# adjerbetian/OpenCL_PathTracer

Hardware: AMD Instinct MI355X
Metric: Msamples/s (paths x bounces) at 1920x1080 (higher is better)
Workload: dtype f32; 1 GPU; BASELINE configs[2]: synthetic random-triangle scene (numpy MT19937 seed 12345): 1000000 triangles (665533 BVH nodes, depth 22), 1920x1080, ray depth 10, JITTERED, 1 light(s); spp_total=256, parallelism=single GPU

## Files before the change

opencl_pathtracer_amd/csrc/kernel_wavefront.hip:

```cpp
#include <hip/hip_runtime.h>

#include "leaf_cull.h"
#include "ptmi_device.hpp"
#include "ptmi_shading.hpp"
#include "ptmi_literal_path.hpp"

#include <atomic>
#include <cstdlib>
#include <cstring>

namespace PTMI_DEV_NS {

constexpr int kWfBlock = 256;
constexpr int kWfBlockNarrow = 64;
constexpr int kWfStack = PTMI_BVH_MAX_DEPTH;
#ifndef PTMI_WF_MIN_WAVES
#define PTMI_WF_MIN_WAVES 5
#endif
#ifndef PTMI_WF_MIN_WAVES_GENERAL
#define PTMI_WF_MIN_WAVES_GENERAL 5
#endif
#ifndef PTMI_WF_QUEUES
#define PTMI_WF_QUEUES 8
#endif
// ... 258 lines not shown
            asm volatile("" ::: "memory");
            Ray wr;
            wr.o = v4(fetch(r.o.x), fetch(r.o.y), fetch(r.o.z), fetch(r.o.w));
            wr.d = v4(fetch(r.d.x), fetch(r.d.y), fetch(r.d.z), fetch(r.d.w));
            wr.ix = wr.iy = wr.iz = 0;
            const float w_limit = fetch(limit);
            if (has_item) {
                unsigned long long* const owner_key = &key_mem[wave_first + owner];
                tri_test<PRE>(e0, e1, [&](float4& l0, float4& l1) { l0 = rec[kL0]; l1 = rec[kL1]; }, wr, w_limit,
                              [&](const V4&, float ray_t, float s, float t, bool front, float nsd) {
                    const bool nan_hit = NANSAFE && !w_shadow && !(nsd == nsd);
                    const unsigned long long key = w_shadow ? ((unsigned long long)w_tri << 32)
                                                   : nan_hit ? 0ull
                                                   : (((unsigned long long)__float_as_uint(nsd) << 32) | (unsigned long long)(~w_tri));
                    atomicMin(owner_key, key);
                    if (!w_shadow && *owner_key == key) {
                        uint32_t* const rec_out = &stack_mem[wave_first + owner];
                        rec_out[0 * kWfBlock] = __float_as_uint(ray_t);
                        rec_out[kWordS * kWfBlock] = __float_as_uint(s);
                        rec_out[kWordT * kWfBlock] = __float_as_uint(t);
                        rec_out[kWordTri * kWfBlock] = w_tri | (front ? kHitFront : 0u) | kHitFound;
                    }
                });
            }
        }
        if (cnt != 0u) {
            const uint32_t won = (uint32_t)(key_mem[tid] >> 32);
            if (NANSAFE && !shadow && won == 0u) {
                give_path_up(radiance, transfer, reflection, p_bbx, p_tri);
                hit_mem[kWordTri * kWfBlock] = 0;
                cur = REF_NONE; tri_i = tri_end = 0; sp = stack_floor;
                if (kTos) tos = REF_NONE;
                job_counter[1] = 1u;
            } else
            if (!shadow) {
                limit = __uint_as_float(won);
                p_tri += cnt; tri_i += cnt;
            } else if (won != 0xFFFFFFFFu) {
                p_tri += won - tri_i + 1u;
                hit_mem[kWordTri * kWfBlock] |= kHitFound;
                tri_end = tri_i; cur = REF_NONE;
            } else {
                p_tri += cnt; tri_i += cnt;
            }
            if (tri_i >= tri_end && ref_is_leaf(cur)) enter_leaf(false);
        }
    };
    auto node_step = [&]() {
        const float4* const rec = reinterpret_cast<const float4*>(&sc.tris[cur & REF_INDEX_MASK_INNER]);
        const float4 a = rec[0], b = rec[1], c = rec[2], d = rec[3];
        const NodeView n = node_view(a, b, c, d);
        const bool fwd = ((dir_signs >> n.axis) & 1u) != 0;
        float d2_1 = 0, d2_2 = 0;
        if (kCull) {
            d2_1 = ptmi_cull::box_distance2(n.lo1, n.hi1, r.o.x, r.o.y, r.o.z);
            d2_2 = ptmi_cull::box_distance2(n.lo2, n.hi2, r.o.x, r.o.y, r.o.z);
            asm volatile("" : "+v"(d2_1), "+v"(d2_2));
        }
        bool h1, h2;
        if (!wave_exact) {
            h1 = box_hit_ordered(n.lo1, n.hi1, r, limit);
            h2 = box_hit_ordered(n.lo2, n.hi2, r, limit);
        } else {
            h1 = box_hit(n.lo1, n.hi1, (n.ref1 & REF_EMPTY) != 0, r, limit);
            h2 = box_hit(n.lo2, n.hi2, (n.ref2 & REF_EMPTY) != 0, r, limit);
        }
        p_bbx += 2;
        bool culled = false;
        if (kCull) {
            const uint32_t cull_bits = n.cull & (dir_signs >> 3) & sc.leaf_cull;
            const bool first = fwd ? h1 : !h2;
            const bool certified = (cull_bits & (first ? ptmi_cull::kCullChild1 : ptmi_cull::kCullChild2)) != 0u;
            culled = (h1 | h2) & certified & ptmi_cull::box_is_beyond(first ? d2_1 : d2_2, limit);
        }
        const uint32_t far_ref = fwd ? n.ref2 : n.ref1;
        sp[kWfBlock] = far_ref;
        uint32_t* const pushed = sp + kWfBlock;
        const uint32_t child = fwd ? (h1 ? n.ref1 : n.ref2) : (h2 ? n.ref2 : n.ref1);
        cur = h1 ? child : (h2 ? child : cur);
        if (kTos) tos = h1 ? (h2 ? far_ref : tos) : tos;
        sp = h1 ? (h2 ? pushed : sp) : sp;
        if (!(h1 | h2)) pop();
        if (ref_is_leaf(cur)) enter_leaf(culled);
    };

    int wait_debt = 0;
    bool pending, want_inner, want_post;
    int n_t, n_i, n_p;
    bool any_lane;
    unsigned long long dead_lanes = 0ull;
    auto survey = [&]() {
        pending = tri_i < tri_end;
        const bool has_node = cur < REF_DEAD;
        const unsigned long long b_t = __builtin_amdgcn_ballot_w64(pending), b_n = __builtin_amdgcn_ballot_w64(has_node), b_dead = dead_lanes;
        const unsigned long long m_t = b_t, m_i = b_n & ~b_t, m_p = ~(b_t | b_n | b_dead);
        want_inner = !pending & has_node;
        want_post = !pending & !has_node & (cur != REF_DEAD);
        any_lane = (m_t | m_i | m_p) != 0ull;
        n_t = __popcll(m_t); n_i = __popcll(m_i); n_p = __popcll(m_p);
        asm volatile("" : "+s"(n_t), "+s"(n_i));
        wait_debt += n_p;
    };
    const int wait_debt_bound = (int)sc.wait_debt;
    auto path_logic_due = [&]() { return n_p > 0 && wait_debt >= wait_debt_bound; };
    auto nothing_traverses = [&]() { return n_t == 0 && n_i == 0; };
    for (;;) {
        survey();
        if (!any_lane) break;
        auto to_path_logic = [&]() { return path_logic_due() || nothing_traverses(); };
        auto pass_is_due = [&]() { return n_t >= kLeafLanes || (n_t > 0 && 3 * n_t >= kLeafRatio * n_i); };
        while (!to_path_logic()) {
            if (pass_is_due()) {
                leaf_pass(pending);
                survey();
                continue;
            }
            if (STATS) { trips_i++; lanes_i += n_i; }
            if (want_inner) node_step();
            survey();
        }
        wait_debt = 0;
        if (STATS) { trips_p++; lanes_p += n_p; }
        const unsigned long long pass_start = STATS ? __builtin_amdgcn_s_memtime() : 0ull;
        bool new_ray = false;
        V4 new_direction = v4(0, 0, 0, 0);
        if (want_post) {
            need_path = cur == REF_IDLE;
            alive = true;
            bool end_path = false, missed = false;
            bool start_shadow = false, do_scatter = false, lit = false;
            Hit hit;
            hit.point = v4(0, 0, 0, 0); hit.s = hit.t = 0; hit.tri = 0; hit.front = false;
            if (!need_path) {
// ... 101 lines not shown
                    got_job = gx < sc.width && gy < sc.height;
                }
            }
            if (open && base + n_want > q_size) {
                q_cur = (q_cur + 1u) % (uint32_t)kQueues;
                q_done++;
            }
        }

        if (want_post) {
            if (got_job) {
                const uint32_t it = first_iteration + it_local * iteration_stride;
                slot = it_local * (sc.width * sc.height) + gy * sc.width + gx;
                seed = lcg_seed(gx, gy, sc.width, sc.height, it, sc.source_seed != 0);
                float sample_x, sample_y;
                draw_sample(sc, gx, gy, it, seed, sample_x, sample_y);
                check(sample_x >= -0.5f && sample_y >= -0.5f && sample_x <= 0.5f && sample_y <= 0.5f, C_CHK_SAMPLE);
                {
                    const DScene& cs = cold_scene();
                    r.o = v4(cs.cam_pos);
                    new_direction = mad(v4(cs.cam_up), sample_y, mad(v4(cs.cam_right), sample_x, v4(cs.cam_dir)));
                }
                radiance = v4(0, 0, 0, 0);
                transfer = v4(1, 1, 1, 1);
                reflection = 0; p_bbx = 0; p_tri = 0;
                in_water = false;
                shadow = false;
                need_path = false;
                bool skip = false;
                if (SS && it > 5u) {
                    const DScene& cs = cold_scene();
                    const uint32_t off = owns_pixel ? gy * sc.width + gx : sample_pixel(sc, sample_x, sample_y);
                    const float n = cs.image_ray_nb[off];
                    const float4 vv = reinterpret_cast<const float4*>(cs.image_v)[off];
                    const float sigma2_n = fmaxf(fmaxf(fdiv(vv.x, n), fdiv(vv.y, n)), fdiv(vv.z, n));
                    uint32_t idx = (uint32_t)n;
                    if (idx > 1000u) idx = 1000u;
                    skip = (double)lcg_random(seed) > (double)fdiv(100 * sigma2_n, cs.x2inv[idx]) + 0.05;
                }
                if (skip) {
                    if (owns_pixel) cold_scene().stage_flag[gy * sc.width + gx] = 0.f;
                    need_path = true;
                } else
                if (sc.max_depth > 0) {
                    limit = INFINITY;
                    new_ray = true;
                } else {
                    finish_path(false);
                }
            }
            if (new_ray) {
                ray_set_direction(r, new_direction);
                dir_signs = (r.d.x > 0 ? 1u : 0u) | (r.d.y > 0 ? 2u : 0u) | (r.d.z > 0 ? 4u : 0u);
                if (kCull && ptmi_cull::ray_may_cull(r.o.x, r.o.y, r.o.z, r.o.w, r.d.w)) dir_signs |= (ptmi_cull::kCullChild1 | ptmi_cull::kCullChild2) << 3;
                const float o_size = __builtin_fabsf(r.o.x) + __builtin_fabsf(r.o.y) + __builtin_fabsf(r.o.z) + __builtin_fabsf(r.o.w);
                const float d_size = __builtin_fabsf(r.d.x) + __builtin_fabsf(r.d.y) + __builtin_fabsf(r.d.z) + __builtin_fabsf(r.d.w);
                bool bad = !((o_size <= 0x1p+40f) & (d_size <= 4.0f));
                if (!PLAIN && !owns_pixel && __builtin_expect(bad, 0)) {
                    const uint32_t place = atomicAdd(&job_counter[2], 1u);
                    bad = place < kGiveUpListCap;
                    if (bad) {
                        job_counter[kGiveUpListFirst + place] = slot;
                        slot |= kGivenUp;
                    }
                }
                if (__builtin_expect(bad, 0)) {
                    give_path_up(radiance, transfer, reflection, p_bbx, p_tri);
                    shadow = false;
                    job_counter[1] = 1u;
                }
                start_query();
                if (__builtin_expect(bad, 0)) { cur = REF_NONE; tri_i = tri_end = 0; }
            }
            if (need_path) cur = alive ? REF_IDLE : REF_DEAD;
        }
        dead_lanes = __builtin_amdgcn_ballot_w64(cur == REF_DEAD);
        wave_exact = __builtin_amdgcn_ballot_w64(exact_boxes) != 0ull;
        if (STATS) cycles_p += __builtin_amdgcn_s_memtime() - pass_start;
    }

    if (STATS && (tid & 63u) == 0) {
        atomicAdd(&block_counters[C_TRIPS_I], (unsigned long long)trips_i);
        atomicAdd(&block_counters[C_LANES_I], lanes_i);
        atomicAdd(&block_counters[C_TRIPS_T], (unsigned long long)(pass_rounds));
        atomicAdd(&block_counters[C_LANES_T], (unsigned long long)pass_items);
        atomicAdd(&block_counters[C_TRIPS_P], (unsigned long long)trips_p);
        atomicAdd(&block_counters[C_LANES_P], lanes_p);
        atomicAdd(&block_counters[C_CYCLES_P], cycles_p);
        atomicAdd(&block_counters[C_CYCLES_LOOP], __builtin_amdgcn_s_memtime() - loop_start);
    }
    if (STATS && culled_items != 0u) atomicAdd(&block_counters[C_LANES_T], (unsigned long long)culled_items);
    if (STATS && item_violations != 0u) atomicAdd(&block_counters[C_ITEM_VIOLATIONS], (unsigned long long)item_violations);
    __syncthreads();
    if (tid < (STATS ? 1u : (uint32_t)PTMI_COUNTER_SPLITS)) {
        unsigned long long* const totals = &block_counters[tid * kSplitWords];
        totals[C_SHADOW] = totals[C_HITS] * sc.n_lights;
    }
    __syncthreads();
    if (STATS) {
        if (tid < C_COUNT) atomicAdd(&cold_scene().counters[tid], block_counters[tid]);
    } else if (tid < kBlockCounters) {
        const uint32_t k = tid / kSplitWords, c = tid % kSplitWords;
        if (k == 0u || block_counters[tid] != 0ull) atomicAdd(&cold_scene().counters[k * C_COUNT + c], block_counters[tid]);
    }
}

template <bool PRE>
// ... 380 lines not shown
```

opencl_pathtracer_amd/csrc/leaf_cull.h:

```cpp
#ifndef PTMI_LEAF_CULL_H
#define PTMI_LEAF_CULL_H

#include <cmath>
#include <cstdint>

#include "ptmi_internal.h"

namespace ptmi_cull {

constexpr float kRel = 1.001f, kAbs = 0.01f, kMaxOrigin = 0x1p+41f;
constexpr double kKappaMax = 0x1p-13, kEpsAbsMax = 2.0e-3;

constexpr uint32_t kCullChild1 = 1u, kCullChild2 = 2u, kCullComputed = 4u;

PTMI_HD float box_distance2(const float lo[3], const float hi[3], float ox, float oy, float oz)
{
    const float dx = fmaxf(fmaxf(lo[0] - ox, ox - hi[0]), 0.0f);
    const float dy = fmaxf(fmaxf(lo[1] - oy, oy - hi[1]), 0.0f);
    const float dz = fmaxf(fmaxf(lo[2] - oz, oz - hi[2]), 0.0f);
    return fmaf(dz, dz, fmaf(dy, dy, dx * dx));
}

PTMI_HD bool ray_may_cull(float ox, float oy, float oz, float ow, float dw)
{
    return fabsf(ox) + fabsf(oy) + fabsf(oz) <= kMaxOrigin && ow == 1.0f && dw == 0.0f;
}
PTMI_HD bool box_is_beyond(float d2, float limit)
{
    return d2 > fmaf(limit, kRel, kAbs);
}
PTMI_HD bool leaf_cull_rule(float d2, float limit, float ox, float oy, float oz, float ow, float dw)
{
    return box_is_beyond(d2, limit) && ray_may_cull(ox, oy, oz, ow, dw);
}

PTMI_HD bool triangle_slack(const ptmi_triangle& t, const float lo[3], const float hi[3], double* eps_abs, double* kappa)
{
    const double u24 = 0x1p-24;
    const float S[3][3] = {{t.s1.x, t.s1.y, t.s1.z}, {t.s2.x, t.s2.y, t.s2.z}, {t.s3.x, t.s3.y, t.s3.z}};
    if (!(t.s1.w == t.s2.w && t.s1.w == t.s3.w && fabsf(t.s1.w) <= 0x1p+20f)) return false;
    if (!(t.n.w == 0.0f || (t.s1.w == 1.0f && fabsf(t.n.w) <= 4.0f))) return false;
    double B2 = 0;
    for (int k = 0; k < 3; k++) {
        if (!(lo[k] <= hi[k] && fabsf(lo[k]) <= 0x1p+20f && fabsf(hi[k]) <= 0x1p+20f)) return false;
        for (int j = 0; j < 3; j++)
            if (!(S[j][k] >= lo[k] && S[j][k] <= hi[k])) return false;
        const double m = fmax(fabs((double)lo[k]), fabs((double)hi[k]));
        B2 += m * m;
    }
    const double B = sqrt(B2);
    const float uf[3] = {S[1][0] - S[0][0], S[1][1] - S[0][1], S[1][2] - S[0][2]}, vf[3] = {S[2][0] - S[0][0], S[2][1] - S[0][1], S[2][2] - S[0][2]};
    const float uv_c = fmaf(uf[2], vf[2], fmaf(uf[1], vf[1], uf[0] * vf[0])), uu_c = fmaf(uf[2], uf[2], fmaf(uf[1], uf[1], uf[0] * uf[0])),
                vv_c = fmaf(vf[2], vf[2], fmaf(vf[1], vf[1], vf[0] * vf[0]));
    const double ud[3] = {uf[0], uf[1], uf[2]}, vd[3] = {vf[0], vf[1], vf[2]};
    const double uu = ud[0] * ud[0] + ud[1] * ud[1] + ud[2] * ud[2], vv = vd[0] * vd[0] + vd[1] * vd[1] + vd[2] * vd[2],
                 uv = ud[0] * vd[0] + ud[1] * vd[1] + ud[2] * vd[2];
    const double lu = sqrt(uu), lv = sqrt(vv);
    if (!(lu >= 0x1p-16 && lv >= 0x1p-16)) return false;
    const double cr[3] = {ud[1] * vd[2] - ud[2] * vd[1], ud[2] * vd[0] - ud[0] * vd[2], ud[0] * vd[1] - ud[1] * vd[0]};
    const double area2 = sqrt(cr[0] * cr[0] + cr[1] * cr[1] + cr[2] * cr[2]);
    if (!(area2 > 0)) return false;
    const double N[3] = {t.n.x, t.n.y, t.n.z};
    const double Nn = (N[0] * cr[0] + N[1] * cr[1] + N[2] * cr[2]) / area2, len_n = sqrt(N[0] * N[0] + N[1] * N[1] + N[2] * N[2]);
    if (!(fabs(Nn) >= 0.25 && len_n <= 4.0)) return false;
    const double tan2 = len_n * len_n - Nn * Nn;
    const double tilt = sqrt(tan2 > 0 ? tan2 : 0) / fabs(Nn);
    if (!(tilt <= 0x1p-18)) return false;
    const float det_c[2] = {uv_c * uv_c - uu_c * vv_c, fmaf(uv_c, uv_c, -(uu_c * vv_c))};
    double dk = 0, c_w = 0;
    for (int m = 0; m < 2; m++) {
        if (!(det_c[m] < 0.0f)) return false;
        const double den = (double)(1.0f / det_c[m]);
        if (!std::isfinite(den)) return false;
// ... 47 lines not shown
```

opencl_pathtracer_amd/csrc/ptmi_api.cpp:

```cpp
#include <cstdlib>
#include <cstring>
#include <mutex>

#include "ptmi_context.h"

using namespace ptmi_internal;

namespace {
std::mutex g_err_mutex;
std::string g_err;
}

void ptmi_internal::set_global_error(const std::string& msg)
{
    std::lock_guard<std::mutex> lock(g_err_mutex);
    g_err = msg;
}

extern "C" {

int ptmi_abi_version(void) { return PTMI_ABI_VERSION; }

int ptmi_device_count(void)
{
// ... 19 lines not shown
        return fail(nullptr, PTMI_ERR_INVALID_ARGUMENT, "config is NULL or struct_size mismatch (ABI)");
    if (cfg->image_width == 0 || cfg->image_height == 0 || (uint64_t)cfg->image_width * cfg->image_height > 0x3FFFFFFFull)
        return fail(nullptr, PTMI_ERR_INVALID_ARGUMENT, "image size must be in [1, 2^30) pixels");
    if (cfg->sampler > PTMI_SAMPLER_UNIFORM) return fail(nullptr, PTMI_ERR_INVALID_ARGUMENT, "unknown sampler");
    if (cfg->lights_size >= PTMI_MAX_LIGHT_SIZE)
        return fail(nullptr, PTMI_ERR_LIMIT, "lights_size >= 30");
    if (cfg->n_devices > PTMI_MAX_DEVICES) return fail(nullptr, PTMI_ERR_INVALID_ARGUMENT, "n_devices > PTMI_MAX_DEVICES");
    if (cfg->super_sampling && (cfg->flags & PTMI_FLAG_MEGAKERNEL))
        return fail(nullptr, PTMI_ERR_UNSUPPORTED, "SUPER_SAMPLING needs the wavefront kernel");

    int n = 0;
    if (hipGetDeviceCount(&n) != hipSuccess || n <= 0)
        return fail(nullptr, PTMI_ERR_NO_DEVICE, "no HIP device available (there is no CPU fallback)");
    std::vector<int> ordinals;
    if (cfg->n_devices <= 1) ordinals.push_back(cfg->n_devices == 1 ? cfg->devices[0] : cfg->device);
    else ordinals.assign(cfg->devices, cfg->devices + cfg->n_devices);
    for (int o : ordinals)
        if (o < 0 || o >= n) return fail(nullptr, PTMI_ERR_NO_DEVICE, "device ordinal out of range");

    ptmi_ctx* ctx = new ptmi_ctx();
    ctx->cfg = *cfg;
    ctx->dev.resize(ordinals.size());
    hipError_t e = hipSuccess;
    for (size_t k = 0; k < ordinals.size() && e == hipSuccess; k++) {
        DeviceState& d = ctx->dev[k];
        d.device = ordinals[k];
        e = hipSetDevice(d.device);
        if (e == hipSuccess) e = hipStreamCreateWithFlags(&d.own_stream, hipStreamNonBlocking);
        if (e == hipSuccess) e = hipStreamCreateWithFlags(&d.copy_stream, hipStreamNonBlocking);
        d.stream = d.own_stream;
        if (e == hipSuccess && k > 0 && d.device != ordinals[0]) {
            (void)hipDeviceEnablePeerAccess(ordinals[0], 0);
            (void)hipGetLastError();
        }
    }
    if (e != hipSuccess) {
        const std::string msg = std::string("device/stream setup: ") + hipGetErrorString(e);
        ptmi_release(ctx);
        return fail(nullptr, PTMI_ERR_HIP, msg);
    }
    {
        const uint64_t tiles = (uint64_t)((cfg->image_width + 7u) / 8u) * ((cfg->image_height + 7u) / 8u);
        const uint64_t by_jobs = (cfg->sampler == PTMI_SAMPLER_RANDOM ? 0x7FFFFFF0ull : 0xFFFFFFF0ull) / (tiles * 64u);
        const uint64_t by_bytes = (4ull << 30) / ((uint64_t)cfg->image_width * cfg->image_height * 20u);
        uint64_t cap = kMaxIterationsPerLaunch;
        if (by_jobs < cap) cap = by_jobs;
        if (by_bytes < cap) cap = by_bytes;
        ctx->iterations_per_launch = cap < 1 ? 1u : (uint32_t)cap;
        if (const char* v = std::getenv("PTMI_ITERATIONS_PER_LAUNCH")) {
            const long want = std::strtol(v, nullptr, 10);
            if (want >= 1 && want <= 32 && (uint32_t)want < ctx->iterations_per_launch) ctx->iterations_per_launch = (uint32_t)want;
        }
    }
    if (const char* v = std::getenv("PTMI_LEAF_CULL")) ctx->leaf_cull = v[0] != '0' ? 1 : 0;
    *out = ctx;
    return PTMI_OK;
}

int ptmi_set_stream(ptmi_ctx* ctx, void* hip_stream)
{
    if (!ctx) return PTMI_ERR_INVALID_ARGUMENT;
    if (ctx->n_dev() != 1) return fail(ctx, PTMI_ERR_UNSUPPORTED, "ptmi_set_stream on a multi-device context");
    DeviceState& d = ctx->dev[0];
    ON_DEVICE(ctx, d);
    HIP_TRY(ctx, hipStreamSynchronize(d.stream));
    if (int rc = fold_events(ctx, d)) return rc;
    d.stream = hip_stream ? (hipStream_t)hip_stream : d.own_stream;
    return PTMI_OK;
}

const char* ptmi_literal_kernel_reason(const ptmi_ctx* ctx)
{
    return ctx && ctx->have_scene && !ctx->literal_kernel_reason.empty() ? ctx->literal_kernel_reason.c_str() : nullptr;
}

int ptmi_synchronize(ptmi_ctx* ctx)
{
    if (!ctx) return PTMI_ERR_INVALID_ARGUMENT;
    for (DeviceState& d : ctx->dev) {
        ON_DEVICE(ctx, d);
        HIP_TRY(ctx, hipStreamSynchronize(d.stream));
    }
    return PTMI_OK;
}

int ptmi_pin_host_buffer(ptmi_ctx* ctx, void* buffer, size_t bytes)
{
    if (!ctx || !buffer || bytes == 0) return PTMI_ERR_INVALID_ARGUMENT;
    if (ctx->host_is_pinned(buffer, bytes)) return PTMI_OK;
    if (ctx->dev.empty()) return PTMI_ERR_STATE;
    ON_DEVICE(ctx, ctx->dev[0]);
    const hipError_t e = hipHostRegister(buffer, bytes, hipHostRegisterPortable);
    if (e != hipSuccess) {
        (void)hipGetLastError();
        return fail(ctx, PTMI_ERR_HIP, std::string("hipHostRegister: ") + hipGetErrorString(e));
    }
    ctx->pinned_host.push_back({(char*)buffer, bytes});
    return PTMI_OK;
}

int ptmi_unpin_host_buffer(ptmi_ctx* ctx, void* buffer)
{
    if (!ctx || !buffer) return PTMI_ERR_INVALID_ARGUMENT;
    for (size_t i = 0; i < ctx->pinned_host.size(); i++) {
        if (ctx->pinned_host[i].p != (char*)buffer) continue;
        for (DeviceState& d : ctx->dev) {
            ON_DEVICE(ctx, d);
// ... 148 lines not shown
```

opencl_pathtracer_amd/csrc/ptmi_device.hpp:

```cpp
#pragma once

#include <hip/hip_runtime.h>

#include "ptmi_detmath.h"
#include "ptmi_internal.h"

#ifndef PTMI_DEFAULT_ARITHMETIC
#define PTMI_DEFAULT_ARITHMETIC 0
#endif
#if PTMI_DEFAULT_ARITHMETIC
#define PTMI_DEV_NS ptmi_dev_da
#define PTMI_ARITH(name) name##_da
#else
#define PTMI_DEV_NS ptmi_dev
#define PTMI_ARITH(name) name
#endif

namespace PTMI_DEV_NS {

using namespace ptmi_internal;

constexpr bool kDefaultArithmetic = PTMI_DEFAULT_ARITHMETIC != 0;

struct V4 {
    float x, y, z, w;
};

__device__ __forceinline__ V4 v4(float x, float y, float z, float w) { return V4{x, y, z, w}; }
__device__ __forceinline__ V4 v4(const float* p) { return V4{p[0], p[1], p[2], p[3]}; }
__device__ __forceinline__ V4 v4(const ptmi_float4& p) { return V4{p.x, p.y, p.z, p.w}; }
__device__ __forceinline__ V4 v4(const float4& p) { return V4{p.x, p.y, p.z, p.w}; }
__device__ __forceinline__ V4 operator+(V4 a, V4 b) { return V4{a.x + b.x, a.y + b.y, a.z + b.z, a.w + b.w}; }
__device__ __forceinline__ V4 operator-(V4 a, V4 b) { return V4{a.x - b.x, a.y - b.y, a.z - b.z, a.w - b.w}; }
__device__ __forceinline__ V4 operator*(V4 a, V4 b) { return V4{a.x * b.x, a.y * b.y, a.z * b.z, a.w * b.w}; }
__device__ __forceinline__ V4 operator*(V4 a, float s) { return V4{a.x * s, a.y * s, a.z * s, a.w * s}; }
__device__ __forceinline__ V4 operator/(V4 a, float s) { return V4{a.x / s, a.y / s, a.z / s, a.w / s}; }
__device__ __forceinline__ V4 operator-(V4 a) { return V4{-a.x, -a.y, -a.z, -a.w}; }

__device__ __forceinline__ float mad(float a, float b, float c)
{
    if (kDefaultArithmetic) return __builtin_fmaf(a, b, c);
    return a * b + c;
}
__device__ __forceinline__ V4 mad(V4 a, V4 b, V4 c) { return V4{mad(a.x, b.x, c.x), mad(a.y, b.y, c.y), mad(a.z, b.z, c.z), mad(a.w, b.w, c.w)}; }
__device__ __forceinline__ V4 mad(V4 a, float s, V4 c) { return V4{mad(a.x, s, c.x), mad(a.y, s, c.y), mad(a.z, s, c.z), mad(a.w, s, c.w)}; }
__device__ __forceinline__ float fdiv(float a, float b)
{
    if (!kDefaultArithmetic) return a / b;
    return __builtin_ldexpf(__builtin_amdgcn_frexp_mantf(a) * __builtin_amdgcn_rcpf(__builtin_amdgcn_frexp_mantf(b)),
                            __builtin_amdgcn_frexp_expf(a) - __builtin_amdgcn_frexp_expf(b));
}
__device__ __forceinline__ float frcp(float b)
{
    if (!kDefaultArithmetic) return 1.0f / b;
    return __builtin_ldexpf(__builtin_amdgcn_rcpf(__builtin_amdgcn_frexp_mantf(b)), -__builtin_amdgcn_frexp_expf(b));
}
struct DivC {
    float c, inv_mant;
// ... 58 lines not shown
        if (d == INFINITY) {
            a = V4{__builtin_copysignf(__builtin_isinf(a.x) ? 1.0f : 0.0f, a.x), __builtin_copysignf(__builtin_isinf(a.y) ? 1.0f : 0.0f, a.y),
                   __builtin_copysignf(__builtin_isinf(a.z) ? 1.0f : 0.0f, a.z), __builtin_copysignf(__builtin_isinf(a.w) ? 1.0f : 0.0f, a.w)};
            d = dot(a, a);
        }
    }
    return a * cl_rsqrt(d);
}
__device__ __forceinline__ V4 cross(V4 a, V4 b)
{
    return V4{__builtin_fmaf(a.y, b.z, b.y * -a.z), __builtin_fmaf(a.z, b.x, b.z * -a.x),
              __builtin_fmaf(a.x, b.y, b.x * -a.y), 0.0f};
}

constexpr float kPi = 3.14159265f;
constexpr float kPiInverse = 0.31830988618f;
constexpr float kMinContribution = 0.001f;
constexpr float kNWater = 1.333f, kNGlass = 1.55f, kNVarnish = 3.f, kSchlick = 0.8f;

struct Ray {
    V4 o, d;
    float ix, iy, iz;
};

__device__ __forceinline__ void ray_set_direction(Ray& r, V4 d)
{
    r.d = normalize(d);
    r.ix = frcp(r.d.x);
    r.iy = frcp(r.d.y);
    r.iz = frcp(r.d.z);
}

__device__ __forceinline__ float lcg_random(int& seed)
{
    seed = (int)((16807u * (uint32_t)seed) & 0x7FFFFFFFu);
    return (float)seed / 2147483648.0f;
}

__device__ __forceinline__ int lcg_seed(uint32_t gx, uint32_t gy, uint32_t w, uint32_t h, uint32_t iteration, bool source_rule = false)
{
    const uint32_t index = gx + gy * w + iteration * w * h;
    uint32_t s = index * 2011u;
    s *= s;
    return (int)((source_rule ? s == 0u : index == 0u) ? 1u : s);
}

__device__ __forceinline__ V4 put_in_same_hemisphere(V4 v, V4 n)
{
    const float d = dot(v, n);
    if (d < 0.001f) v = mad(n, 0.01f - d, v);
    return v;
}

__device__ __forceinline__ bool box_hit(const float lo[3], const float hi[3], bool is_empty, const Ray& r, float limit)
{
    const bool px = r.d.x > 0, py = r.d.y > 0, pz = r.d.z > 0;
    float tmin = ((px ? lo[0] : hi[0]) - r.o.x) * r.ix;
    float tmax = ((px ? hi[0] : lo[0]) - r.o.x) * r.ix;
    bool miss = (tmin < 0) & (tmax < 0);
    const float tymin = ((py ? lo[1] : hi[1]) - r.o.y) * r.iy;
    const float tymax = ((py ? hi[1] : lo[1]) - r.o.y) * r.iy;
    miss |= (tymin < 0) & (tymax < 0);
    miss |= (tmin > tymax) | (tymin > tmax);
    tmin = tymin > tmin ? tymin : tmin;
    tmax = tymax < tmax ? tymax : tmax;
    const float tzmin = ((pz ? lo[2] : hi[2]) - r.o.z) * r.iz;
    const float tzmax = ((pz ? hi[2] : lo[2]) - r.o.z) * r.iz;
    miss |= (tzmin < 0) & (tzmax < 0);
    miss |= (tmin > tzmax) | (tzmin > tmax);
    tmin = tzmin > tmin ? tzmin : tmin;
    miss |= !(tmin < 0) & (tmin > limit);
    return !(miss | is_empty);
}

typedef float ptmi_f2 __attribute__((ext_vector_type(2)));
__device__ __forceinline__ bool box_hit_ordered(const float lo[3], const float hi[3], const Ray& r, float limit)
{
    const bool px = r.d.x > 0, py = r.d.y > 0, pz = r.d.z > 0;
    const ptmi_f2 o_xy = {r.o.x, r.o.y}, i_xy = {r.ix, r.iy}, o_zz = {r.o.z, r.o.z}, i_zz = {r.iz, r.iz};
    const ptmi_f2 near_xy = {px ? lo[0] : hi[0], py ? lo[1] : hi[1]}, far_xy = {px ? hi[0] : lo[0], py ? hi[1] : lo[1]};
    const ptmi_f2 z_nf = {pz ? lo[2] : hi[2], pz ? hi[2] : lo[2]};
    const ptmi_f2 tn = (near_xy - o_xy) * i_xy, tf = (far_xy - o_xy) * i_xy, tz = (z_nf - o_zz) * i_zz;
    const float tmin = __builtin_fmaxf(__builtin_fmaxf(tn.x, tn.y), tz.x);
    const float tmax = __builtin_fminf(__builtin_fminf(tf.x, tf.y), tz.y);
    return !((tmax < 0) | (tmin > tmax) | (tmin > limit));
}
__device__ __forceinline__ bool ray_slabs_are_ordered(const Ray& r)
{
    return (__builtin_fabsf(r.ix) < INFINITY) & (__builtin_fabsf(r.iy) < INFINITY) & (__builtin_fabsf(r.iz) < INFINITY) &
           (__builtin_fabsf(r.o.x) < INFINITY) & (__builtin_fabsf(r.o.y) < INFINITY) & (__builtin_fabsf(r.o.z) < INFINITY);
}

struct NodeView {
    float lo1[3], hi1[3], lo2[3], hi2[3];
    uint32_t ref1, ref2, axis, cull;
};
__device__ __forceinline__ NodeView node_view(const float4 a, const float4 b, const float4 c, const float4 d)
{
    return NodeView{{a.x, a.y, a.z}, {a.w, b.x, b.y}, {b.z, b.w, c.x}, {c.y, c.z, c.w},
                    __float_as_uint(d.x), __float_as_uint(d.y), __float_as_uint(d.z), __float_as_uint(d.w)};
}

struct Hit {
    V4 point;
    float s, t;
    uint32_t tri;
    bool front;
};
__device__ __forceinline__ Hit no_hit() { return Hit{v4(0, 0, 0, 0), 0.f, 0.f, 0u, false}; }

__device__ __forceinline__ bool tri_hit(const V4 S1, const V4 S2, const V4 S3, const V4 N, const Ray& r, float& limit,
                                        Hit& h)
{
    const V4 u = S2 - S1;
    const V4 v = S3 - S1;
    const float d = dot(N, S1);
    const float nd = dot(N, r.d);
    if ((nd > -0.00001f) && (nd < 0.00001f)) return false;
    const V4 q = mad(r.d, fdiv(d - dot(N, r.o), nd), r.o);
    const V4 full = q - r.o;
    const float nsd = dot(full, full);
    if (nsd > limit) return false;
    if (nsd < 0.00001f) return false;
    const V4 w = q - S1;
    const float uv = dot(u, v), wv = dot(w, v), wu = dot(w, u), uu = dot(u, u), vv = dot(v, v);
    const float denom = frcp(mad(uv, uv, -(uu * vv)));
    const float s = mad(uv, wv, -(vv * wu)) * denom;
    const float t = mad(uv, wu, -(uu * wv)) * denom;
    if (s < 0 || t < 0 || s + t > 1) return false;
    if (dot(full, r.d) < 0) return false;
    limit = nsd;
    h.point = q;
    h.s = s;
    h.t = t;
    h.front = nd < 0;
// ... 221 lines not shown
```

opencl_pathtracer_amd/csrc/ptmi_scene_memory.cpp:

```cpp
#include <algorithm>
#include <chrono>
#include <cstdlib>
#include <cstring>

#include "leaf_cull.h"
#include "ptmi_context.h"
#include "scene_layout.h"

using namespace ptmi_internal;

bool ptmi_internal::one_path_per_lane(const ptmi_ctx* ctx)
{
    if ((ctx->cfg.flags & PTMI_FLAG_MEGAKERNEL) != 0) return true;
    if (ctx->literal_kernel_reason.empty()) return false;
    const char* force = std::getenv("PTMI_LITERAL_KERNEL");
    return ctx->cfg.sampler == PTMI_SAMPLER_RANDOM || (force && force[0] == '1');
}

int ptmi_internal::quiesce(ptmi_ctx* ctx, DeviceState& d)
{
    ON_DEVICE(ctx, d);
    d.schedule.forget();
    for (int i = 0; i < kStageSets; i++)
        if (d.launch_stream[i]) HIP_TRY(ctx, hipStreamSynchronize(d.launch_stream[i]));
// ... 94 lines not shown
    if (int rc = upload(ctx, d, lay.mats, &ds.mats)) return rc;
    if (int rc = upload(ctx, d, lay.big_leaves, &ds.big_leaves)) return rc;
    if (int rc = upload(ctx, d, sc->lights, sc->lights_size, &ds.lights)) return rc;
    if (int rc = upload(ctx, d, sc->textures, sc->textures_size, &ds.textures)) return rc;
    if (int rc = upload(ctx, d, sc->textures_data, sc->textures_data_size, &ds.texels)) return rc;

    constexpr size_t kCounterBlock = ((C_COUNT * 8 + 255) / 256) * 256, kSceneBlock = ((sizeof(DScene) + 255) / 256) * 256;
    constexpr size_t kSetCounterBlock = ((PTMI_COUNTER_SPLITS * C_COUNT * 8 + 255) / 256) * 256;
    constexpr int kSets = kStageSets;
    char *dk = nullptr, *dsc = nullptr;
    if (int rc = scene_alloc(ctx, d, ctx->color_bytes(), d.d_color)) return rc;
    if (int rc = scene_alloc(ctx, d, ctx->count_bytes(), d.d_count)) return rc;
    if (int rc = scene_alloc(ctx, d, ctx->hist_words() * 4, d.d_hist)) return rc;
    if (int rc = scene_alloc(ctx, d, kCounterBlock + 256 + kSets * 8 * 1024 * 4 + kSets * kSetCounterBlock, dk)) return rc;
    if (int rc = scene_alloc(ctx, d, (1 + kSets) * kSceneBlock, dsc)) return rc;
    d.d_scene = (DScene*)dsc;
    d.d_counters = (unsigned long long*)dk;
    d.d_job_counter = (uint32_t*)(dk + kCounterBlock);
    for (int i = 0; i < kSets; i++) {
        d.d_set_counters[i] = (unsigned long long*)(dk + kCounterBlock + kSets * 8 * 1024 * 4 + i * kSetCounterBlock);
        d.d_scene_set[i] = (DScene*)(dsc + (1 + i) * kSceneBlock);
    }

    ds.image_color = d.d_color;
    ds.image_ray_nb = d.d_count;
    const bool hist = !(ctx->cfg.flags & PTMI_FLAG_NO_HISTOGRAMS);
    ds.hist_depths = hist ? d.d_hist : nullptr;
    ds.hist_bbx = hist ? d.d_hist + ctx->cfg.ray_max_depth + 1 : nullptr;
    ds.hist_tri = hist ? d.d_hist + ctx->cfg.ray_max_depth + 1 + PTMI_MAX_INTERSECTION_NUMBER : nullptr;
    ds.counters = d.d_counters;
    ds.super_sampling = ctx->cfg.super_sampling ? 1u : 0u;
    if (ds.super_sampling) {
        float* dx = nullptr;
        if (int rc = scene_alloc(ctx, d, ctx->color_bytes(), ds.image_v)) return rc;
        if (int rc = scene_alloc(ctx, d, sizeof kX2inv, dx)) return rc;
        if (int rc = scene_alloc(ctx, d, ctx->count_bytes(), ds.stage_flag)) return rc;
        HIP_TRY(ctx, hipMemcpy(dx, kX2inv, sizeof kX2inv, hipMemcpyHostToDevice));
        ds.x2inv = dx;
    }
    ds.sky = *sc->sky;
    std::memcpy(ds.cam_pos, &sc->camera_position, 16);
    std::memcpy(ds.cam_dir, &sc->camera_direction, 16);
    std::memcpy(ds.cam_right, &sc->camera_right, 16);
    std::memcpy(ds.cam_up, &sc->camera_up, 16);
    ds.tris_precomputed = lay.tris_precomputed ? 1u : 0u;
    ds.plain_shading = lay.plain_shading ? 1u : 0u;
    ds.nan_safe = lay.literal_kernel_reason.empty() ? 0u : 1u;
    ds.nan_walk_box_tests = lay.nan_walk_box_tests; ds.nan_walk_tri_tests = lay.nan_walk_tri_tests; ds.nan_walk_last_tri = lay.nan_walk_last_tri;
    if (std::getenv("PTMI_WALK_NAN_RAYS") != nullptr) ds.nan_walk_box_tests = ds.nan_walk_tri_tests = 0xFFFFFFFFu;
    ds.boxes_ordered = (lay.boxes_ordered && std::getenv("PTMI_GENERIC_BOXES") == nullptr) ? 1u : 0u;
    constexpr uint32_t kCullMinLeaves = 1024;
    const bool cull_bits = lay.tris_precomputed && lay.literal_kernel_reason.empty();
    const bool cull = ctx->leaf_cull < 0 ? lay.cullable_leaves >= kCullMinLeaves : ctx->leaf_cull != 0;
    ds.leaf_cull = (cull && cull_bits) ? (ptmi_cull::kCullChild1 | ptmi_cull::kCullChild2) : 0u;
    ds.root_ref = lay.root_ref;
    ds.width = ctx->cfg.image_width;
    ds.height = ctx->cfg.image_height;
    ds.max_depth = ctx->cfg.ray_max_depth;
    ds.n_lights = ctx->cfg.lights_size;
    ds.sampler = ctx->cfg.sampler;
    ds.russian_roulette = (ctx->cfg.flags & PTMI_FLAG_RUSSIAN_ROULETTE) ? 1u : 0u;
    ds.source_seed = (ctx->cfg.flags & PTMI_FLAG_SOURCE_SEED) ? 1u : 0u;
    return upload_scene_records(ctx, d);
}

}

extern "C" {

int ptmi_initialize_memory(ptmi_ctx* ctx, const ptmi_scene* sc)
{
    if (!ctx) return PTMI_ERR_INVALID_ARGUMENT;
    if (!sc || sc->struct_size != sizeof(ptmi_scene))
        return fail(ctx, PTMI_ERR_INVALID_ARGUMENT, "scene is NULL or struct_size mismatch (ABI)");
    free_scene_memory(ctx);

    Relayout lay;
    if (int rc = build_layout(ctx, sc, lay)) return rc;
    ctx->literal_kernel_reason = lay.literal_kernel_reason;
    if (one_path_per_lane(ctx) && !(ctx->cfg.flags & PTMI_FLAG_MEGAKERNEL) && ctx->cfg.super_sampling) {
        ctx->literal_kernel_reason.clear();
        return fail(ctx, PTMI_ERR_UNSUPPORTED, "SUPER_SAMPLING needs the wavefront kernel, which cannot reproduce the reference on this scene with "
                                               "the RANDOM sampler: " + lay.literal_kernel_reason);
    }
    ctx->stack_levels = lay.max_depth < 1 ? 1 : lay.max_depth;
    ctx->update.triangulation_size = sc->triangulation_size;
    ctx->update.n_big_leaves = (uint32_t)lay.big_leaves.size();
    ctx->update.tris_precomputed = lay.tris_precomputed;
    ctx->update.material_is_simple_color = lay.material_is_simple_color;
    for (DeviceState& d : ctx->dev)
        if (int rc = upload_scene(ctx, d, lay, sc)) {
            const std::string msg = ctx->err;
            free_scene_memory(ctx);
            ctx->err = msg;
            return rc;
        }
    ctx->have_scene = true;
    if (int rc = ptmi_clear(ctx)) return rc;
    return ptmi_synchronize(ctx);
}

int ptmi_clear(ptmi_ctx* ctx)
{
    NEED_SCENE(ctx);
    for (DeviceState& d : ctx->dev) {
        ON_DEVICE(ctx, d);
        HIP_TRY(ctx, hipMemsetAsync(d.ds.image_color, 0, ctx->color_bytes(), d.stream));
// ... 216 lines not shown
```

Before: 1005 Msamples/s.

## Fuse box distance into slab test and cull certified far children before pushing

Computes the squared box-to-origin distance from the slab differences already formed in the ray-box test, using a med3 instruction instead of a separate box_distance2 pass. Also extends leaf culling to the far child: when both children are hit and the far child is a certified leaf lying beyond the current hit distance, it is not pushed on the traversal stack, and its triangle count is credited to the sample counter. This is enabled by default for non-shadow rays via a new kCullPushed bit, which reuses the kCullComputed bit value. It aims to cut stack traffic and later leaf visits. The risk is wrong culling if kCullComputed is not a valid per-node certification for the far child.

```diff
diff --git a/opencl_pathtracer_amd/csrc/kernel_wavefront.hip b/opencl_pathtracer_amd/csrc/kernel_wavefront.hip
--- a/opencl_pathtracer_amd/csrc/kernel_wavefront.hip
+++ b/opencl_pathtracer_amd/csrc/kernel_wavefront.hip
@@ -334,33 +334,35 @@
         const NodeView n = node_view(a, b, c, d);
         const bool fwd = ((dir_signs >> n.axis) & 1u) != 0;
         float d2_1 = 0, d2_2 = 0;
-        if (kCull) {
-            d2_1 = ptmi_cull::box_distance2(n.lo1, n.hi1, r.o.x, r.o.y, r.o.z);
-            d2_2 = ptmi_cull::box_distance2(n.lo2, n.hi2, r.o.x, r.o.y, r.o.z);
-            asm volatile("" : "+v"(d2_1), "+v"(d2_2));
-        }
         bool h1, h2;
         if (!wave_exact) {
-            h1 = box_hit_ordered(n.lo1, n.hi1, r, limit);
-            h2 = box_hit_ordered(n.lo2, n.hi2, r, limit);
+            h1 = box_hit_ordered(n.lo1, n.hi1, r, limit, kCull ? &d2_1 : nullptr);
+            if (kCull) asm volatile("" : "+v"(d2_1));
+            h2 = box_hit_ordered(n.lo2, n.hi2, r, limit, kCull ? &d2_2 : nullptr);
         } else {
-            h1 = box_hit(n.lo1, n.hi1, (n.ref1 & REF_EMPTY) != 0, r, limit);
-            h2 = box_hit(n.lo2, n.hi2, (n.ref2 & REF_EMPTY) != 0, r, limit);
+            h1 = box_hit(n.lo1, n.hi1, (n.ref1 & REF_EMPTY) != 0, r, limit, kCull ? &d2_1 : nullptr);
+            h2 = box_hit(n.lo2, n.hi2, (n.ref2 & REF_EMPTY) != 0, r, limit, kCull ? &d2_2 : nullptr);
         }
         p_bbx += 2;
-        bool culled = false;
+        bool culled = false, far_counted = false;
         if (kCull) {
             const uint32_t cull_bits = n.cull & (dir_signs >> 3) & sc.leaf_cull;
             const bool first = fwd ? h1 : !h2;
             const bool certified = (cull_bits & (first ? ptmi_cull::kCullChild1 : ptmi_cull::kCullChild2)) != 0u;
             culled = (h1 | h2) & certified & ptmi_cull::box_is_beyond(first ? d2_1 : d2_2, limit);
+            const bool far_certified = (cull_bits & ptmi_cull::kCullPushed) != 0u && (cull_bits & (fwd ? ptmi_cull::kCullChild2 : ptmi_cull::kCullChild1)) != 0u;
+            far_counted = h1 & h2 & far_certified & ptmi_cull::box_is_beyond(fwd ? d2_2 : d2_1, limit);
         }
         const uint32_t far_ref = fwd ? n.ref2 : n.ref1;
         sp[kWfBlock] = far_ref;
-        uint32_t* const pushed = sp + kWfBlock;
+        uint32_t* const pushed = far_counted ? sp : sp + kWfBlock;
         const uint32_t child = fwd ? (h1 ? n.ref1 : n.ref2) : (h2 ? n.ref2 : n.ref1);
+        if (kCull && far_counted) {
+            p_tri += ref_leaf_count(far_ref);
+            if (STATS) culled_items += ref_leaf_count(far_ref);
+        }
         cur = h1 ? child : (h2 ? child : cur);
-        if (kTos) tos = h1 ? (h2 ? far_ref : tos) : tos;
+        if (kTos) tos = h1 ? (h2 ? (far_counted ? tos : far_ref) : tos) : tos;
         sp = h1 ? (h2 ? pushed : sp) : sp;
         if (!(h1 | h2)) pop();
         if (ref_is_leaf(cur)) enter_leaf(culled);
@@ -568,7 +570,8 @@
             if (new_ray) {
                 ray_set_direction(r, new_direction);
                 dir_signs = (r.d.x > 0 ? 1u : 0u) | (r.d.y > 0 ? 2u : 0u) | (r.d.z > 0 ? 4u : 0u);
-                if (kCull && ptmi_cull::ray_may_cull(r.o.x, r.o.y, r.o.z, r.o.w, r.d.w)) dir_signs |= (ptmi_cull::kCullChild1 | ptmi_cull::kCullChild2) << 3;
+                if (kCull && ptmi_cull::ray_may_cull(r.o.x, r.o.y, r.o.z, r.o.w, r.d.w))
+                    dir_signs |= (ptmi_cull::kCullChild1 | ptmi_cull::kCullChild2 | (shadow ? 0u : ptmi_cull::kCullPushed)) << 3;
                 const float o_size = __builtin_fabsf(r.o.x) + __builtin_fabsf(r.o.y) + __builtin_fabsf(r.o.z) + __builtin_fabsf(r.o.w);
                 const float d_size = __builtin_fabsf(r.d.x) + __builtin_fabsf(r.d.y) + __builtin_fabsf(r.d.z) + __builtin_fabsf(r.d.w);
                 bool bad = !((o_size <= 0x1p+40f) & (d_size <= 4.0f));
diff --git a/opencl_pathtracer_amd/csrc/leaf_cull.h b/opencl_pathtracer_amd/csrc/leaf_cull.h
--- a/opencl_pathtracer_amd/csrc/leaf_cull.h
+++ b/opencl_pathtracer_amd/csrc/leaf_cull.h
@@ -12,6 +12,7 @@
 constexpr double kKappaMax = 0x1p-13, kEpsAbsMax = 2.0e-3;
 
 constexpr uint32_t kCullChild1 = 1u, kCullChild2 = 2u, kCullComputed = 4u;
+constexpr uint32_t kCullPushed = kCullComputed;
 
 PTMI_HD float box_distance2(const float lo[3], const float hi[3], float ox, float oy, float oz)
 {
@@ -19,6 +20,20 @@
     const float dy = fmaxf(fmaxf(lo[1] - oy, oy - hi[1]), 0.0f);
     const float dz = fmaxf(fmaxf(lo[2] - oz, oz - hi[2]), 0.0f);
     return fmaf(dz, dz, fmaf(dy, dy, dx * dx));
+}
+
+PTMI_HD float median_with_zero(float a, float b)
+{
+#if defined(__HIP_DEVICE_COMPILE__)
+    return __builtin_amdgcn_fmed3f(a, 0.0f, b);
+#else
+    return fmaxf(fminf(a, b), fminf(fmaxf(a, b), 0.0f));
+#endif
+}
+PTMI_HD float box_distance2_from_slabs(float ax, float bx, float ay, float by, float az, float bz)
+{
+    const float mx = median_with_zero(ax, bx), my = median_with_zero(ay, by), mz = median_with_zero(az, bz);
+    return fmaf(mz, mz, fmaf(my, my, mx * mx));
 }
 
 PTMI_HD bool ray_may_cull(float ox, float oy, float oz, float ow, float dw)
diff --git a/opencl_pathtracer_amd/csrc/ptmi_api.cpp b/opencl_pathtracer_amd/csrc/ptmi_api.cpp
--- a/opencl_pathtracer_amd/csrc/ptmi_api.cpp
+++ b/opencl_pathtracer_amd/csrc/ptmi_api.cpp
@@ -95,7 +95,7 @@
             if (want >= 1 && want <= 32 && (uint32_t)want < ctx->iterations_per_launch) ctx->iterations_per_launch = (uint32_t)want;
         }
     }
-    if (const char* v = std::getenv("PTMI_LEAF_CULL")) ctx->leaf_cull = v[0] != '0' ? 1 : 0;
+    if (const char* v = std::getenv("PTMI_LEAF_CULL")) ctx->leaf_cull = v[0] == '0' ? 0 : v[0] == '2' ? 2 : 1;
     *out = ctx;
     return PTMI_OK;
 }
diff --git a/opencl_pathtracer_amd/csrc/ptmi_device.hpp b/opencl_pathtracer_amd/csrc/ptmi_device.hpp
--- a/opencl_pathtracer_amd/csrc/ptmi_device.hpp
+++ b/opencl_pathtracer_amd/csrc/ptmi_device.hpp
@@ -4,6 +4,7 @@
 
 #include "ptmi_detmath.h"
 #include "ptmi_internal.h"
+#include "leaf_cull.h"
 
 #ifndef PTMI_DEFAULT_ARITHMETIC
 #define PTMI_DEFAULT_ARITHMETIC 0
@@ -168,20 +169,24 @@
     return v;
 }
 
-__device__ __forceinline__ bool box_hit(const float lo[3], const float hi[3], bool is_empty, const Ray& r, float limit)
+__device__ __forceinline__ bool box_hit(const float lo[3], const float hi[3], bool is_empty, const Ray& r, float limit, float* distance2 = nullptr)
 {
     const bool px = r.d.x > 0, py = r.d.y > 0, pz = r.d.z > 0;
-    float tmin = ((px ? lo[0] : hi[0]) - r.o.x) * r.ix;
-    float tmax = ((px ? hi[0] : lo[0]) - r.o.x) * r.ix;
+    const float xn = (px ? lo[0] : hi[0]) - r.o.x, xf = (px ? hi[0] : lo[0]) - r.o.x;
+    const float yn = (py ? lo[1] : hi[1]) - r.o.y, yf = (py ? hi[1] : lo[1]) - r.o.y;
+    const float zn = (pz ? lo[2] : hi[2]) - r.o.z, zf = (pz ? hi[2] : lo[2]) - r.o.z;
+    if (distance2) *distance2 = ptmi_cull::box_distance2_from_slabs(xn, xf, yn, yf, zn, zf);
+    float tmin = xn * r.ix;
+    float tmax = xf * r.ix;
     bool miss = (tmin < 0) & (tmax < 0);
-    const float tymin = ((py ? lo[1] : hi[1]) - r.o.y) * r.iy;
-    const float tymax = ((py ? hi[1] : lo[1]) - r.o.y) * r.iy;
+    const float tymin = yn * r.iy;
+    const float tymax = yf * r.iy;
     miss |= (tymin < 0) & (tymax < 0);
     miss |= (tmin > tymax) | (tymin > tmax);
     tmin = tymin > tmin ? tymin : tmin;
     tmax = tymax < tmax ? tymax : tmax;
-    const float tzmin = ((pz ? lo[2] : hi[2]) - r.o.z) * r.iz;
-    const float tzmax = ((pz ? hi[2] : lo[2]) - r.o.z) * r.iz;
+    const float tzmin = zn * r.iz;
+    const float tzmax = zf * r.iz;
     miss |= (tzmin < 0) & (tzmax < 0);
     miss |= (tmin > tzmax) | (tzmin > tmax);
     tmin = tzmin > tmin ? tzmin : tmin;
@@ -190,13 +195,15 @@
 }
 
 typedef float ptmi_f2 __attribute__((ext_vector_type(2)));
-__device__ __forceinline__ bool box_hit_ordered(const float lo[3], const float hi[3], const Ray& r, float limit)
+__device__ __forceinline__ bool box_hit_ordered(const float lo[3], const float hi[3], const Ray& r, float limit, float* distance2 = nullptr)
 {
     const bool px = r.d.x > 0, py = r.d.y > 0, pz = r.d.z > 0;
     const ptmi_f2 o_xy = {r.o.x, r.o.y}, i_xy = {r.ix, r.iy}, o_zz = {r.o.z, r.o.z}, i_zz = {r.iz, r.iz};
     const ptmi_f2 near_xy = {px ? lo[0] : hi[0], py ? lo[1] : hi[1]}, far_xy = {px ? hi[0] : lo[0], py ? hi[1] : lo[1]};
     const ptmi_f2 z_nf = {pz ? lo[2] : hi[2], pz ? hi[2] : lo[2]};
-    const ptmi_f2 tn = (near_xy - o_xy) * i_xy, tf = (far_xy - o_xy) * i_xy, tz = (z_nf - o_zz) * i_zz;
+    const ptmi_f2 dn = near_xy - o_xy, df = far_xy - o_xy, dz = z_nf - o_zz;
+    if (distance2) *distance2 = ptmi_cull::box_distance2_from_slabs(dn.x, df.x, dn.y, df.y, dz.x, dz.y);
+    const ptmi_f2 tn = dn * i_xy, tf = df * i_xy, tz = dz * i_zz;
     const float tmin = __builtin_fmaxf(__builtin_fmaxf(tn.x, tn.y), tz.x);
     const float tmax = __builtin_fminf(__builtin_fminf(tf.x, tf.y), tz.y);
     return !((tmax < 0) | (tmin > tmax) | (tmin > limit));
diff --git a/opencl_pathtracer_amd/csrc/ptmi_scene_memory.cpp b/opencl_pathtracer_amd/csrc/ptmi_scene_memory.cpp
--- a/opencl_pathtracer_amd/csrc/ptmi_scene_memory.cpp
+++ b/opencl_pathtracer_amd/csrc/ptmi_scene_memory.cpp
@@ -170,7 +170,7 @@
     constexpr uint32_t kCullMinLeaves = 1024;
     const bool cull_bits = lay.tris_precomputed && lay.literal_kernel_reason.empty();
     const bool cull = ctx->leaf_cull < 0 ? lay.cullable_leaves >= kCullMinLeaves : ctx->leaf_cull != 0;
-    ds.leaf_cull = (cull && cull_bits) ? (ptmi_cull::kCullChild1 | ptmi_cull::kCullChild2) : 0u;
+    ds.leaf_cull = (cull && cull_bits) ? (ptmi_cull::kCullChild1 | ptmi_cull::kCullChild2 | (ctx->leaf_cull == 1 ? 0u : ptmi_cull::kCullPushed)) : 0u;
     ds.root_ref = lay.root_ref;
     ds.width = ctx->cfg.image_width;
     ds.height = ctx->cfg.image_height;
```

Result: faster. 1028 Msamples/s, median of 6 (+2.3%).
